# lefarov/Ape-X-DQN

Measured on AMD Instinct MI355X. Metric: learner grad-steps/sec at batch 512, 84x84x4 dueling DQN, higher is better.
Workload: dtype fp32; 1 GPU; model=dueling NatureCNN (reference DuellingDQN, conv1=64), 4x84x84, A=4, global_batch=512, seq_len=1, parallelism=dp1, batch_scope=global, per_rank_rows=512, replay_per_gpu=100000, learner=fused/hip, hip_graphs=True

## Files before the change

apex_dqn_amd/csrc/sumtree.hip:

```cpp
#include "apex_common.h"
#include <stdlib.h>
#include "head_common.h"
#include "igemm_wgrad.h"
#include "rmsprop_common.h"
#include "pack_rows.h"

#define APEX_DBG_SITES 8
#ifdef APEX_DEBUG_BOUNDS
__device__ int apex_dbg_count[APEX_DBG_SITES];
__device__ long long apex_dbg_first[APEX_DBG_SITES];
__device__ __forceinline__ bool apex_dbg_ok(int64_t i, int64_t n, int site) {
  if (i >= 0 && i < n) return true;
  if (atomicAdd(&apex_dbg_count[site], 1) == 0) apex_dbg_first[site] = (long long)i;
  return false;
}
#define APEX_DBG_OK(i, n, site) apex_dbg_ok((int64_t)(i), (int64_t)(n), site)
#define APEX_DBG_CLAMP(i, n, site) (APEX_DBG_OK(i, n, site) ? (i) : ((i) < 0 ? 0 : (n) - 1))
#else
#define APEX_DBG_OK(i, n, site) true
#define APEX_DBG_CLAMP(i, n, site) (i)
#endif

struct TreeDesc {
  float* leaf;
// ... 525 lines not shown
  if (n <= 0 && ctr_to_bump == nullptr) return 0;
  if (dedupe && n > 1024) return (int)hipErrorInvalidValue;
  const int threads = n <= 1024 ? ((n + 63) / 64) * 64 : 1024;
  const int nb = n > 0 ? blocks_for(n, threads) : 1;
  tree_update_kernel<<<nb, threads > 0 ? threads : 64, 0, st>>>(t, idx, values, n, mode, alpha, eps, gen_expect,
                                                               gen, dedupe, ctr_to_bump, tree_kfirst(t));
  APEX_CHECK_LAUNCH();
}

APEX_EXPORT int apex_tree_zero_range(TreeDesc t, int64_t start, int64_t count, hipStream_t st) {
  if (count <= 0) return 0;
  tree_zero_range_kernel<<<blocks_for(count, 256), 256, 0, st>>>(t, start, count, tree_kfirst(t));
  APEX_CHECK_LAUNCH();
}

APEX_EXPORT int apex_replay_insert(TreeDesc t, RecordDesc r, int64_t start, int K, const int32_t* s_obs,
                                   const int32_t* s_nxt, const int32_t* s_act, const float* s_rew,
                                   const float* s_gam, const float* s_prio, float alpha, float eps,
                                   hipStream_t st) {
  if (K <= 0) return 0;
  replay_insert_kernel<<<blocks_for(K, 256), 256, 0, st>>>(t, r, start, K, s_obs, s_nxt, s_act, s_rew,
                                                           s_gam, s_prio, alpha, eps, tree_kfirst(t));
  APEX_CHECK_LAUNCH();
}

APEX_EXPORT int apex_tree_sample(TreeDesc t, RecordDesc r, int B, uint64_t seed, const uint64_t* ctr,
                                 float beta, int64_t* out_idx, float* out_w,
                                 int32_t* out_gen, int32_t* out_obs, int32_t* out_nxt, int32_t* out_act,
                                 float* out_rew, float* out_gam, int32_t* out_nxt2, const double* shard_stats,
                                 int shard_rank, int shard_world, uint64_t shard_seed, float* out_wscale,
                                 int64_t mcap, hipStream_t st) {
  if (B <= 0) return 0;
  if (mcap <= 0) mcap = (int64_t)shard_world * B;
  if (shard_stats != nullptr && (B < 3 || shard_world < 1 || shard_rank < 0 || shard_rank >= shard_world))
    return (int)hipErrorInvalidValue;
  const int waves_per_block = 4;
  tree_sample_kernel<<<blocks_for(B, waves_per_block), 64 * waves_per_block, 0, st>>>(
      SampleArgs{t, r, B, seed, ctr, beta, out_idx, out_w, out_gen, out_obs, out_nxt, out_act,
                 out_rew, out_gam, out_nxt2, shard_stats, shard_rank, shard_world, shard_seed, out_wscale,
                 mcap});
  APEX_CHECK_LAUNCH();
}

APEX_EXPORT int apex_tree_rebuild(TreeDesc t, hipStream_t st) {
  fill_u32_kernel<<<1, 64, 0, st>>>(t.min_bits, 0x7f800000u, 1);
  for (int k = 1; k <= t.L; ++k) {
    int64_t nd = t.n[k];
    const int wpb = 4;
    if (k == 1) {
      const int nb = blocks_for(nd, wpb);
      tree_reduce_leaf_kernel<<<nb < 512 ? nb : 512, 64 * wpb, 0, st>>>(t.leaf, t.n[0], t.nodes + t.off[1], nd,
                                                                       t.min_bits);
      continue;
    }
    tree_reduce_level_kernel<<<blocks_for(nd, wpb), 64 * wpb, 0, st>>>(
        nullptr, t.nodes + t.off[k - 1], t.n[k - 1], t.nodes + t.off[k], nd, t.min_bits);
  }
  APEX_CHECK_LAUNCH();
}

APEX_EXPORT int apex_gather_frames(const uint8_t* ring, const int32_t* slots, int n_slots, int64_t nframes,
                                   int64_t frame_bytes, uint8_t* out, hipStream_t st) {
  if (n_slots <= 0) return 0;
  if (frame_bytes % 16) return (int)hipErrorInvalidValue;
  gather_frames_kernel<<<n_slots, 256, 0, st>>>(ring, slots, nframes, frame_bytes, out);
  APEX_CHECK_LAUNCH();
}

__global__ void fill16_kernel(uint4* p, int64_t n, int nt) {
  typedef uint32_t u32x4v __attribute__((ext_vector_type(4)));
  const uint4 v = make_uint4(1u, 1u, 1u, 1u);
  const u32x4v vv = {1u, 1u, 1u, 1u};
  for (int64_t i = (int64_t)blockIdx.x * blockDim.x + threadIdx.x; i < n; i += (int64_t)gridDim.x * blockDim.x) {
    if (nt) __builtin_nontemporal_store(vv, reinterpret_cast<u32x4v*>(p + i));
    else p[i] = v;
  }
}

APEX_EXPORT int apex_fill16(void* p, int64_t n, int nt, hipStream_t st) {
  fill16_kernel<<<2048, 256, 0, st>>>(reinterpret_cast<uint4*>(p), n, nt);
  APEX_CHECK_LAUNCH();
}

APEX_EXPORT int apex_abi_version() { return 8; }

APEX_EXPORT int apex_debug_bounds_enabled() {
#ifdef APEX_DEBUG_BOUNDS
  return 1;
#else
  return 0;
#endif
}

APEX_EXPORT int apex_debug_errors(int* counts, long long* first, int reset) {
#ifdef APEX_DEBUG_BOUNDS
  hipError_t e = hipDeviceSynchronize();
  if (e != hipSuccess) return (int)e;
  e = hipMemcpyFromSymbol(counts, HIP_SYMBOL(apex_dbg_count), sizeof(int) * APEX_DBG_SITES);
  if (e != hipSuccess) return (int)e;
  e = hipMemcpyFromSymbol(first, HIP_SYMBOL(apex_dbg_first), sizeof(long long) * APEX_DBG_SITES);
  if (e != hipSuccess) return (int)e;
  if (reset) {
    int zc[APEX_DBG_SITES] = {0};
    long long zf[APEX_DBG_SITES] = {0};
    hipMemcpyToSymbol(HIP_SYMBOL(apex_dbg_count), zc, sizeof(zc));
    e = hipMemcpyToSymbol(HIP_SYMBOL(apex_dbg_first), zf, sizeof(zf));
  }
  return (int)e;
#else
  for (int i = 0; i < APEX_DBG_SITES; ++i) {
    counts[i] = 0;
    first[i] = 0;
  }
  return 0;
#endif
}

APEX_EXPORT int apex_rmsprop_sample(float* p, const float* g, float* v, float* m, bf16_t* pb, int64_t n,
                                    const double* partials, int npart, float lr, float alpha, float eps_opt,
                                    float clip, int centered, float* norm_out, TreeDesc t, RecordDesc r, int B,
                                    uint64_t seed, const uint64_t* ctr, float beta,
                                    int64_t* out_idx, float* out_w, int32_t* out_gen, int32_t* out_obs,
                                    int32_t* out_nxt, int32_t* out_act, float* out_rew, float* out_gam,
                                    int32_t* out_nxt2, const double* shard_stats, int shard_rank, int shard_world,
                                    uint64_t shard_seed, float* out_wscale, int64_t mcap, bf16_t* pb_lo,
                                    const double* wnorm, int wn, int wstride, CfFragOut fo, const RmsSegs* seg,
                                    const float* gpre, int64_t npre, hipStream_t st) {
  if (mcap <= 0) mcap = (int64_t)shard_world * B;
  if (shard_stats != nullptr && (B < 3 || shard_world < 1 || shard_rank < 0 || shard_rank >= shard_world))
    return (int)hipErrorInvalidValue;
  if (((uintptr_t)p | (uintptr_t)g | (uintptr_t)v | (uintptr_t)m) & 15) return (int)hipErrorInvalidValue;
  if ((((uintptr_t)pb | (uintptr_t)pb_lo) & 7) || B < 0) return (int)hipErrorInvalidValue;
  constexpr int nt = 512, maxb = 256;
  int nb = (int)((n / 4 + nt - 1) / nt);
  nb = nb < 1 ? 1 : (nb > maxb ? maxb : nb);
  RmsSegs sg{};
  if (seg != nullptr) {
    sg = *seg;
    if (sg.nseg < 1 || sg.nseg > 3) return (int)hipErrorInvalidValue;
    int64_t tot = 0;
    for (int k = 0; k < sg.nseg; ++k) {
      if ((sg.off[k] & 3) || sg.len[k] <= 0 || sg.off[k] < 0 || sg.off[k] + sg.len[k] > n)
        return (int)hipErrorInvalidValue;
      tot += sg.len[k];
    }
    const int64_t fend = fo.c3f != nullptr && fo.w3_off + 36864 > fo.w2_off + 65536 ? fo.w3_off + 36864
                                                                                     : fo.w2_off + 65536;
    const int64_t need0 = fo.w1frag != nullptr ? fend / 4 / nt + 1 : 1;
    int b0 = 0;
    for (int k = 0; k < sg.nseg; ++k) {
      const int64_t full = (sg.len[k] / 4 + nt - 1) / nt;
      int64_t nbk = (int64_t)maxb * sg.len[k] / tot;
      if (k == 0 && nbk < need0) nbk = need0;
      if (nbk > full) nbk = full;
      if (nbk < 1) nbk = 1;
      sg.blk0[k] = b0;
      b0 += (int)nbk;
    }
    sg.blk0[sg.nseg] = b0;
    nb = sg.blk0[1];
  }
  const int nsb = B > 0 ? blocks_for(B, nt / 64) : 0;
  const int64_t n0 = seg != nullptr ? sg.len[0] : n;
  if (fo.w1frag != nullptr && (seg != nullptr && sg.off[0] != 0)) return (int)hipErrorInvalidValue;
  if (fo.w1frag != nullptr && (fo.c2f == nullptr || (fo.C != 1 && fo.C != 2 && fo.C != 4) ||
                               (fo.w1_off & 3) || (fo.w2_off & 7) || fo.w1_off + 4096LL * fo.C > n0 ||
                               fo.w2_off + 65536 > n0 ||
// ... 65 lines not shown
```

apex_dqn_amd/ops/_lib.py:

```python
from __future__ import annotations

import ctypes
import os
from typing import Optional

import torch

from . import build as _build

c_p = ctypes.c_void_p
c_i = ctypes.c_int
c_i64 = ctypes.c_int64
c_u64 = ctypes.c_uint64
c_f = ctypes.c_float


class TreeDesc(ctypes.Structure):
    _fields_ = [("leaf", c_p), ("nodes", c_p), ("off", c_i64 * 8), ("n", c_i64 * 8), ("L", c_i),
                ("min_bits", c_p)]


class RecordDesc(ctypes.Structure):
    _fields_ = [("obs", c_p), ("nxt", c_p), ("act", c_p), ("rew", c_p), ("gam", c_p), ("gen", c_p),
                ("C", c_i), ("cap", c_i64), ("nframes", c_i64)]
# ... 57 lines not shown
                ("nsplit", c_i), ("nb", c_i), ("s2dC", c_i), ("Kc", c_i), ("scale", c_f), ("blk0", c_i),
                ("cpb", c_i), ("jnorm", c_p)]


class FinalizeDesc(ctypes.Structure):
    _fields_ = [("job", RedJob * 4), ("njobs", c_i), ("nrm_n", c_i), ("nrm_ptr", c_p), ("norm_part", c_p),
                ("norm_slot0", c_i), ("nblocks", c_i)]


class Conv1WgDesc(ctypes.Structure):
    _fields_ = [("ring", c_p), ("slots", c_p), ("dy", c_p), ("slab", c_p), ("bias_slab", c_p), ("zero16", c_p),
                ("N", c_i), ("C", c_i), ("dy_lo", c_p), ("wq", c_p)]


class Conv1S2DDesc(ctypes.Structure):
    _fields_ = [("ring", c_p), ("slots", c_p), ("w", c_p), ("w2", c_p), ("bias", c_p), ("bias2", c_p),
                ("y", c_p), ("zero16", c_p), ("scratch", c_p), ("N", c_i), ("C", c_i), ("m_switch", c_i),
                ("in_scale", c_f), ("probe", c_p), ("w32", c_p), ("w2_32", c_p), ("y_lo", c_p),
                ("c2f_src", c_p * 4), ("c2f_out", c_p), ("c2f_bf16", c_i)]


_SIGS = {
    "apex_abi_version": ([], c_i),
    "apex_build_id": ([], ctypes.c_char_p),
    "apex_fill16": ([c_p, c_i64, c_i, c_p], c_i),
    "apex_tree_update": ([TreeDesc, c_p, c_p, c_i, c_i, c_f, c_f, c_p, c_p, c_i, c_p, c_p], c_i),
    "apex_tree_zero_range": ([TreeDesc, c_i64, c_i64, c_p], c_i),
    "apex_replay_insert": ([TreeDesc, RecordDesc, c_i64, c_i, c_p, c_p, c_p, c_p, c_p, c_p, c_f, c_f, c_p],
                           c_i),
    "apex_tree_sample": ([TreeDesc, RecordDesc, c_i, c_u64, c_p, c_f, c_p, c_p, c_p, c_p, c_p, c_p, c_p,
                          c_p, c_p, c_p, c_i, c_i, c_u64, c_p, c_i64, c_p], c_i),
    "apex_tree_rebuild": ([TreeDesc, c_p], c_i),
    "apex_gather_frames": ([c_p, c_p, c_i, c_i64, c_i64, c_p, c_p], c_i),
    "apex_debug_bounds_enabled": ([], c_i),
    "apex_debug_errors": ([c_p, c_p, c_i], c_i),
    "apex_grad_sqnorm_partials": ([c_p, c_i64, c_p, c_p], c_i),
    "apex_rmsprop_step": ([c_p, c_p, c_p, c_p, c_p, c_i64, c_p, c_f, c_f, c_f, c_f, c_i, c_p, c_p, c_p, c_i, c_i,
                           c_p], c_i),
    "apex_cast_bf16": ([c_p, c_p, c_i64, c_p, c_p], c_i),
    "apex_spin_hold": ([c_i, c_i, c_i, c_p, c_p], c_i),
    "apex_rmsprop_step_np": ([c_p, c_p, c_p, c_p, c_p, c_i64, c_p, c_i, c_f, c_f, c_f, c_f, c_i, c_p, c_p, c_p,
                              c_i, c_i, c_p], c_i),
    "apex_grad_finalize": ([FinalizeDesc, c_p], c_i),
    "apex_norm_total": ([c_p, c_i, c_p, c_p], c_i),
    "apex_ddqn_head": ([c_p, c_p, HeadParams, HeadParams, c_p, c_p, c_p, c_p, c_i, c_i, c_i, c_f, c_f, c_p,
                        c_p, c_p, c_p, c_p, c_p, c_i, c_i, HeadLo, HeadPart, C2dPack, IsNorm, c_p], c_i),
    "apex_rmsprop_sample": ([c_p, c_p, c_p, c_p, c_p, c_i64, c_p, c_i, c_f, c_f, c_f, c_f, c_i, c_p,
                             TreeDesc, RecordDesc, c_i, c_u64, c_p, c_f, c_p, c_p, c_p, c_p, c_p, c_p, c_p, c_p,
                             c_p, c_p, c_i, c_i, c_u64, c_p, c_i64, c_p, c_p, c_i, c_i, CfFragOut, c_p, c_p, c_i64,
                             c_p], c_i),
    "apex_head_wgrad_prio": ([c_p, c_p, c_i, c_i, c_p, c_p, c_p, c_p, c_i, TreeDesc, c_p, c_p, c_p, c_p, c_f, c_f,
                              c_p, c_p, c_p, c_p, c_p, c_p, c_i, c_i, c_p, c_i64, c_p], c_i),
    "apex_fc_wgrad_head_prio": ([WgradDesc, c_p, c_p, c_i, c_i, c_p, c_p, c_p, c_p, c_i, TreeDesc, c_p, c_p, c_p,
                                 c_p, c_f, c_f, c_p, c_p, c_p, c_p], c_i),
    "apex_head_wgrad": ([c_p, c_p, c_i, c_i, c_p, c_p, c_p, c_p, c_i, c_p, c_p], c_i),
    "apex_actor_head": ([c_p, HeadParams, c_i, c_i, c_p, c_u64, c_p, c_p, c_p, c_i, c_p, c_p], c_i),
    "apex_conv1_s2d_fwd": ([Conv1S2DDesc, c_i, c_p], c_i),
    "apex_conv1_wgrad_img": ([Conv1WgDesc, c_i, c_p], c_i),
    "apex_slab_reduce": ([c_p, c_i, c_i64, c_f, c_p, c_p, c_i, c_p, c_i, c_i, c_p], c_i),
    "apex_s2d_pack_w1": ([c_p, c_p, c_i, c_p], c_i),
    "apex_s2d_unpack_w1_grad": ([c_p, c_p, c_i, c_p], c_i),
    "apex_s2d_frames": ([c_p, c_p, c_i64, c_i64, c_i64, c_p], c_i),
    "apex_atari_frames": ([c_p, c_p, c_i64, c_i64, c_i64, c_p], c_i),
    "apex_pack_rows": ([c_p, c_p, c_p, c_i, c_i, c_p, c_i64, c_p], c_i),
    "apex_sqnorm_ranges": ([c_p, c_i64, c_p, c_i64, c_p, c_i, c_p], c_i),
    "apex_copy_segments": ([c_i, c_p, c_p, c_p, c_p], c_i),
}

_LIB: Optional[ctypes.CDLL] = None
_LOAD_ERROR: Optional[str] = None


def _declare(lib: ctypes.CDLL) -> None:
    for name, (args, res) in _SIGS.items():
        fn = getattr(lib, name, None)
        if fn is None:
            continue
        fn.argtypes = args
        fn.restype = res
    from . import conv_sigs
    conv_sigs.declare(lib)


ABI_VERSION = 8


def load(build_if_missing: bool = True) -> Optional[ctypes.CDLL]:
    global _LIB, _LOAD_ERROR
    if _LIB is not None:
        return _LIB
    debug = debug_bounds_requested()
    try:
        path = _build.ensure_current("kernels_debug" if debug else "kernels", allow_build=build_if_missing)
        lib = ctypes.CDLL(path, mode=ctypes.RTLD_LOCAL)
        _declare(lib)
        if lib.apex_abi_version() != ABI_VERSION:
            raise RuntimeError(f"{path}: ABI {lib.apex_abi_version()} != {ABI_VERSION}")
        _LIB = lib
    except Exception as e:
        _LOAD_ERROR = repr(e)
        _LIB = None
    return _LIB


def debug_bounds_requested() -> bool:
    return os.environ.get("APEX_DEBUG_BOUNDS", "0") not in ("", "0")


DEBUG_SITES = ("tree_update.leaf", "replay_insert.slot", "tree_sample.slot", "gather_frames.frame",
               "replay_insert.frame_value", "tree_zero_range.slot", "unused6", "unused7")


def debug_errors(reset: bool = True) -> dict:
    lib = require_kernels()
    counts = (ctypes.c_int * 8)()
    first = (ctypes.c_longlong * 8)()
    check(lib.apex_debug_errors(ctypes.addressof(counts), ctypes.addressof(first), int(reset)), "debug_errors")
    return {DEBUG_SITES[i]: (int(counts[i]), int(first[i])) for i in range(8) if counts[i]}


def available() -> bool:
    return load() is not None


def require_kernels() -> ctypes.CDLL:
    lib = load()
    if lib is None:
        raise RuntimeError(f"apex HIP kernel library unavailable: {_LOAD_ERROR}. "
                           f"Run `python -m apex_dqn_amd.ops.build`.")
    return lib


def stream_ptr(device: Optional[torch.device] = None) -> int:
    return torch.cuda.current_stream(device).cuda_stream


def ptr(t: Optional[torch.Tensor]) -> Optional[int]:
    return None if t is None else t.data_ptr()


def head_lo(Hon_lo=None, Htg_lo=None, dH_lo=None) -> HeadLo:
    lo = HeadLo()
    lo.Hon, lo.Htg, lo.dH = ptr(Hon_lo), ptr(Htg_lo), ptr(dH_lo)
    return lo


def check(rc: int, what: str) -> None:
    if rc != 0:
        raise RuntimeError(f"{what} failed with hipError {rc}")
```

apex_dqn_amd/ops/conv.py:

```python
from __future__ import annotations

from typing import Dict, Optional, Tuple


import torch

from . import _lib
from .switches import SW


class Workspace:
    def __init__(self):
        self.bufs: Dict[Tuple, torch.Tensor] = {}

    def get(self, key, numel: int, device, dtype=torch.float32) -> torch.Tensor:
        k = (key, numel, str(device), dtype)
        t = self.bufs.get(k)
        if t is None:
            t = torch.empty(numel, dtype=dtype, device=device)
            self.bufs[k] = t
        return t

    work_queue = False

# ... 324 lines not shown
def conv3_dgrad_img(lib, dy: torch.Tensor, w3: torch.Tensor, mask: torch.Tensor, out: torch.Tensor,
                    grid: int = 0) -> None:
    from .conv_sigs import Conv3DgradImgDesc
    N = dy.shape[0]
    assert tuple(dy.shape) == (N, 7, 7, 64) and tuple(out.shape) == (N, 9, 9, 64)
    assert tuple(mask.shape) == (N, 9, 9, 64) and tuple(w3.shape) == (64, 3, 3, 64)
    assert dy.is_contiguous() and out.is_contiguous() and mask.is_contiguous() and w3.is_contiguous()
    d = Conv3DgradImgDesc()
    d.dy, d.w, d.mask, d.dx, d.N = dy.data_ptr(), w3.data_ptr(), mask.data_ptr(), out.data_ptr(), N
    _lib.check(lib.apex_conv3_dgrad_img(d, int(grid), _lib.stream_ptr()), "conv3_dgrad_img")


def conv3_dgrad(lib, dy: torch.Tensor, w3: torch.Tensor, mask: torch.Tensor, out: torch.Tensor, dy_lo=None,
                w_lo=None, out_lo=None) -> None:
    N = dy.shape[0]
    assert w3.shape == (64, 3, 3, 64)
    if SW.conv3_dgrad_img and dy_lo is None and hasattr(lib, "apex_conv3_dgrad_img"):
        conv3_dgrad_img(lib, dy, w3, mask, out)
        return
    d = _conv_desc(x=dy.data_ptr(), w=w3.data_ptr(), y=out.data_ptr(), mask=mask.data_ptr(), N=N, H=7, W=7,
                   Cin=64, OH=9, OW=9, Cout=64, KH=3, KW=3, stride=1, pad=2, mode=1, K=576,
                   bt=1, ldb=576, koff=_KOFF3, **_lo(dy_lo, w_lo, None, out_lo))
    _launch_fwd(lib, d)


def conv2_dgrad_img(lib, dy: torch.Tensor, w2: torch.Tensor, mask: torch.Tensor, out: torch.Tensor,
                    grid: int = 0, dy_lo=None, w_lo=None, out_lo=None, ws: Optional["Workspace"] = None,
                    packed: bool = False) -> None:
    from .conv_sigs import Conv2DgradImgDesc
    N = dy.shape[0]
    assert tuple(dy.shape) == (N, 9, 9, 64) and tuple(out.shape) == (N, 20, 20, 64)
    assert tuple(mask.shape) == (N, 20, 20, 64) and tuple(w2.shape) == (64, 4, 4, 64)
    assert dy.is_contiguous() and out.is_contiguous() and mask.is_contiguous() and w2.is_contiguous()
    d = Conv2DgradImgDesc()
    d.dy, d.w, d.mask, d.dx, d.N = dy.data_ptr(), w2.data_ptr(), mask.data_ptr(), out.data_ptr(), N
    if dy_lo is not None:
        for t in (dy_lo, w_lo, out_lo):
            assert t is not None and t.is_contiguous() and t.dtype == torch.bfloat16
        d.dy_lo, d.w_lo, d.dx_lo = dy_lo.data_ptr(), w_lo.data_ptr(), out_lo.data_ptr()
    ws = ws if ws is not None else _DEFAULT_WS
    d.wfrag = c2d_wfrag_buffer(ws, dy.device).data_ptr()
    d.wfrag_ready = int(packed)
    d.wq = ws.wq(("c2d_wq", N, int(grid)), dy.device)
    d.cls_split = int(dy_lo is not None and N <= SW.conv2_dgrad_cls_max)
    _lib.check(lib.apex_conv2_dgrad_img(d, int(grid), _lib.stream_ptr()), "conv2_dgrad_img")


def conv2_dgrad(lib, dy: torch.Tensor, w2: torch.Tensor, mask: torch.Tensor, out: torch.Tensor, dy_lo=None,
                w_lo=None, out_lo=None, ws: Optional["Workspace"] = None, packed: bool = False) -> None:
    N = dy.shape[0]
    assert w2.shape == (64, 4, 4, 64)
    if SW.conv2_dgrad_img and hasattr(lib, "apex_conv2_dgrad_img"):
        conv2_dgrad_img(lib, dy, w2, mask, out, dy_lo=dy_lo, w_lo=w_lo, out_lo=out_lo, ws=ws, packed=packed)
        return
    d = _conv_desc(x=dy.data_ptr(), w=w2.data_ptr(), y=out.data_ptr(), mask=mask.data_ptr(), N=N, H=9, W=9,
                   Cin=64, OH=10, OW=10, Cout=64, KH=2, KW=2, stride=1, pad=1, mode=1, K=256, ncls=4,
                   ostride=2, OHfull=20, OWfull=20, bt=1, ldb=1024, koff=_KOFF2, **_lo(dy_lo, w_lo, None, out_lo))
    _launch_fwd(lib, d)


def _wg_desc(**kw) -> "_lib.WgradDesc":
    d = _lib.WgradDesc()
    d.dy, d.x, d.frame_slots = kw["dy"], kw["x"], kw.get("frame_slots")
    d.slab, d.bias_slab = kw["slab"], kw.get("bias_slab")
    d.N, d.H, d.W, d.Cin = kw.get("N", 1), kw.get("H", 1), kw.get("W", 1), kw.get("Cin", 64)
    d.OH, d.OW, d.KH, d.KW = kw.get("OH", 1), kw.get("OW", 1), kw.get("KH", 1), kw.get("KW", 1)
    d.stride, d.pad_h, d.pad_w, d.mode = kw.get("stride", 1), 0, 0, kw["mode"]
    d.Co, d.Kc, d.ldd, d.ldx = kw["Co"], kw["Kc"], kw["ldd"], kw.get("ldx", 0)
    d.rows_per_split, d.Mred = kw["rows_per_split"], kw["Mred"]
    d.norm_part, d.norm_slot0 = kw.get("norm_part"), kw.get("norm_slot0", 0)
    d.dy_lo, d.x_lo = kw.get("dy_lo"), kw.get("x_lo")
    return d


_WG_ROWS = 64
_WG_TBL = 1024


def _splits(Mred: int, target_rows: int, max_rows: int) -> Tuple[int, int]:
    rows = max(_WG_ROWS, min(max_rows, (target_rows // _WG_ROWS) * _WG_ROWS))
    return (Mred + rows - 1) // rows, rows


def conv_wgrad(lib, ws: Workspace, dy: torch.Tensor, x: torch.Tensor, KH: int, stride: int,
               dw_out: torch.Tensor, db_out: torch.Tensor, target_rows: int = 0, jobs: Optional[list] = None,
               dy_lo=None, x_lo=None) -> None:
    N, OH, OW, Co = dy.shape
    if target_rows <= 0:
        small = N < 256
        target_rows = {3: SW.wg_rows3, 4: SW.wg_rows2}.get(KH) or \
            ((192 if small else 384) if KH == 3 else (352 if small else 704))
    _, H, W, Cin = x.shape
    Kc = KH * KH * Cin
    Mred = N * OH * OW
    nsplit, rows = _splits(Mred, target_rows, _WG_TBL)
    slab = ws.get(("wg", Co, Kc), nsplit * Co * Kc, dy.device)
    bslab = ws.get(("wgb", Co, Kc), nsplit * Co, dy.device)
    d = _wg_desc(dy=dy.data_ptr(), x=x.data_ptr(), slab=slab.data_ptr(), bias_slab=bslab.data_ptr(), N=N,
                 H=H, W=W, Cin=Cin, OH=OH, OW=OW, KH=KH, KW=KH, stride=stride, mode=1, Co=Co, Kc=Kc, ldd=Co,
                 rows_per_split=rows, Mred=Mred, dy_lo=_lib.ptr(dy_lo), x_lo=_lib.ptr(x_lo))
    if jobs is not None:
        _lib.check(lib.apex_conv_wgrad(d, None, None, nsplit, 1.0, _lib.stream_ptr()), "conv_wgrad")
        jobs.append(dict(slab=slab, bslab=bslab, out=dw_out, bout=db_out, n=Co * Kc, nsplit=nsplit, nb=Co,
                         s2dC=0, Kc=Kc, scale=1.0))
        return
    _lib.check(lib.apex_conv_wgrad(d, dw_out.data_ptr(), db_out.data_ptr(), nsplit, 1.0, _lib.stream_ptr()),
               "conv_wgrad")


def conv1_wgrad_ring(lib, ws: Workspace, dy: torch.Tensor, ring: torch.Tensor, slots: torch.Tensor,
                     scale: float, dw_out: torch.Tensor, db_out: torch.Tensor, grid: int = 0,
                     jobs: Optional[list] = None, dy_lo: Optional[torch.Tensor] = None) -> None:
    N, OH, OW, Co = dy.shape
    C = slots.shape[1]
    assert (OH, OW, Co) == (20, 20, 64) and slots.dtype == torch.int32 and dy.is_contiguous()
    G = grid if grid > 0 else min(N, 256)
    K = 64 * C
    slab = ws.get(("wg1img", C, G), G * 64 * K, dy.device)
    bslab = ws.get(("wg1imgb", G), G * 64, dy.device)
    zero = ws.get(("zero16",), 64, ring.device, torch.uint8)
    if not getattr(ws, "_zeroed", False):
        zero.zero_()
        ws._zeroed = True
    d = _lib.Conv1WgDesc()
    d.ring, d.slots, d.dy = ring.data_ptr(), slots.data_ptr(), dy.data_ptr()
    d.slab, d.bias_slab, d.zero16 = slab.data_ptr(), bslab.data_ptr(), zero.data_ptr()
    d.N, d.C = N, C
    d.dy_lo = _lib.ptr(dy_lo)
    d.wq = ws.wq(("c1w_wq", N, int(G)), dy.device)
    st = _lib.stream_ptr()
    _lib.check(lib.apex_conv1_wgrad_img(d, G, st), "conv1_wgrad_img")
    if jobs is not None:
        jobs.append(dict(slab=slab, bslab=bslab, out=dw_out, bout=db_out, n=64 * K, nsplit=G, nb=64, s2dC=C, Kc=K,
                         scale=float(scale)))
        return
    _lib.check(lib.apex_slab_reduce(slab.data_ptr(), G, 64 * K, float(scale), dw_out.data_ptr(), bslab.data_ptr(),
                                    64, db_out.data_ptr(), C, K, st), "slab_reduce")


def conv2_dgrad_conv1_wgrad_fused(lib, ws: Workspace, dy: torch.Tensor, dy_lo: torch.Tensor, w2: torch.Tensor,
                                  w_lo: torch.Tensor, mask: torch.Tensor, ring: torch.Tensor, slots: torch.Tensor,
                                  scale: float, dw_out: torch.Tensor, db_out: torch.Tensor, grid: int = 0,
                                  jobs: Optional[list] = None, packed: bool = False,
                                  dx: Optional[torch.Tensor] = None, dx_lo: Optional[torch.Tensor] = None,
                                  wq: int = 0) -> None:
    from .conv_sigs import Conv21BwdDesc
    N = dy.shape[0]
    C = slots.shape[1]
    assert tuple(dy.shape) == (N, 9, 9, 64) and tuple(mask.shape) == (N, 20, 20, 64)
    assert tuple(w2.shape) == (64, 4, 4, 64) and slots.dtype == torch.int32 and slots.shape[0] == N
    assert dy.is_contiguous() and mask.is_contiguous() and w2.is_contiguous() and slots.is_contiguous()
    for t in (dy_lo, w_lo):
        assert t is not None and t.is_contiguous() and t.dtype == torch.bfloat16
    for t in (dx, dx_lo):
        assert t is None or (tuple(t.shape) == (N, 20, 20, 64) and t.is_contiguous() and t.dtype == torch.bfloat16)
    G = grid if grid > 0 else min(N, 256)
    K = 64 * C
    slab = ws.get(("wg1img", C, G), G * 64 * K, dy.device)
    bslab = ws.get(("wg1imgb", G), G * 64, dy.device)
    zero = ws.get(("zero16",), 64, ring.device, torch.uint8)
    if not getattr(ws, "_zeroed", False):
        zero.zero_()
        ws._zeroed = True
    d = Conv21BwdDesc()
    d.dy, d.dy_lo, d.w, d.w_lo, d.mask = dy.data_ptr(), dy_lo.data_ptr(), w2.data_ptr(), w_lo.data_ptr(), mask.data_ptr()
    d.wfrag = c2d_wfrag_buffer(ws, dy.device).data_ptr()
    d.wfrag_ready = int(packed)
    d.ring, d.slots, d.zero16 = ring.data_ptr(), slots.data_ptr(), zero.data_ptr()
    d.slab, d.bias_slab = slab.data_ptr(), bslab.data_ptr()
    d.dx, d.dx_lo = _lib.ptr(dx), _lib.ptr(dx_lo)
    d.wq = wq or None
    d.N, d.C = N, C
    st = _lib.stream_ptr()
    _lib.check(lib.apex_conv21_bwd_fused(d, G, st), "conv21_bwd_fused")
    if jobs is not None:
        jobs.append(dict(slab=slab, bslab=bslab, out=dw_out, bout=db_out, n=64 * K, nsplit=G, nb=64, s2dC=C, Kc=K,
                         scale=float(scale)))
        return
    _lib.check(lib.apex_slab_reduce(slab.data_ptr(), G, 64 * K, float(scale), dw_out.data_ptr(), bslab.data_ptr(),
                                    64, db_out.data_ptr(), C, K, st), "slab_reduce")


def conv1_wgrad_ring_tiled(lib, ws: Workspace, dy: torch.Tensor, ring: torch.Tensor, slots: torch.Tensor,
                           scale: float, dw_out: torch.Tensor, db_out: torch.Tensor, target_rows: int = 0,
                           jobs: Optional[list] = None, dy_lo: Optional[torch.Tensor] = None) -> None:
    if target_rows <= 0:
        target_rows = 800 if dy_lo is not None else 1024
    N, OH, OW, Co = dy.shape
    C = slots.shape[1]
    Kc = C * 64
# ... 131 lines not shown
```

apex_dqn_amd/ops/conv_sigs.py:

```python
from __future__ import annotations

import ctypes

c_p = ctypes.c_void_p
c_i = ctypes.c_int
c_i64 = ctypes.c_int64
c_f = ctypes.c_float


class Conv2ImgDesc(ctypes.Structure):
    _fields_ = [("x", c_p), ("w", c_p), ("w2", c_p), ("bias", c_p), ("bias2", c_p), ("y", c_p),
                ("N", c_i), ("img_switch", c_i), ("x_lo", c_p), ("w_lo", c_p), ("w2_lo", c_p), ("y_lo", c_p),
                ("wfrag", c_p), ("wfrag_ready", c_i)]


class Conv12Desc(ctypes.Structure):
    _fields_ = [("ring", c_p), ("slots", c_p), ("w1", c_p), ("w1b", c_p), ("b1", c_p), ("b1b", c_p),
                ("w2", c_p), ("w2_lo", c_p), ("w2b", c_p), ("w2b_lo", c_p), ("wfrag", c_p), ("pack_sets", c_i),
                ("b2", c_p), ("b2b", c_p), ("y1", c_p), ("y1_lo", c_p), ("y2", c_p), ("y2_lo", c_p),
                ("w1frag", c_p), ("scratch", c_p), ("N", c_i), ("C", c_i), ("img_switch", c_i), ("copy_n", c_i),
                ("in_scale", ctypes.c_float), ("probe", c_p), ("wq", c_p), ("bf16", c_i), ("probe_split", c_i),
                ("w3", c_p), ("w3_lo", c_p), ("w3b", c_p), ("w3b_lo", c_p), ("b3", c_p), ("b3b", c_p),
                ("y3", c_p), ("y3_lo", c_p), ("w3frag", c_p)]


class Conv2DgradImgDesc(ctypes.Structure):
    _fields_ = [("dy", c_p), ("w", c_p), ("mask", c_p), ("dx", c_p), ("N", c_i), ("dy_lo", c_p), ("w_lo", c_p),
                ("dx_lo", c_p), ("wfrag", c_p), ("wfrag_ready", c_i), ("wq", c_p), ("cls_split", c_i)]


class Conv21BwdDesc(ctypes.Structure):
    _fields_ = [("dy", c_p), ("dy_lo", c_p), ("w", c_p), ("w_lo", c_p), ("mask", c_p), ("wfrag", c_p),
                ("wfrag_ready", c_i), ("ring", c_p), ("slots", c_p), ("zero16", c_p), ("slab", c_p),
                ("bias_slab", c_p), ("dx", c_p), ("dx_lo", c_p), ("wq", c_p), ("N", c_i), ("C", c_i)]


class C2dPackJob(ctypes.Structure):
    _fields_ = [("w", c_p), ("w_lo", c_p), ("out", c_p)]


class Conv3DgradImgDesc(ctypes.Structure):
    _fields_ = [("dy", c_p), ("w", c_p), ("mask", c_p), ("dx", c_p), ("N", c_i)]


def declare(lib: ctypes.CDLL) -> None:
    from ._lib import ConvDesc, WgradDesc
    sigs = {
        "apex_conv2_img_fwd": ([Conv2ImgDesc, c_i, c_p], c_i),
        "apex_conv12_fused_fwd": ([Conv12Desc, c_i, c_p], c_i),
        "apex_conv12_pack": ([Conv12Desc, c_p], c_i),
        "apex_conv2_dgrad_img": ([Conv2DgradImgDesc, c_i, c_p], c_i),
        "apex_conv3_dgrad_img": ([Conv3DgradImgDesc, c_i, c_p], c_i),
        "apex_conv21_bwd_fused": ([Conv21BwdDesc, c_i, c_p], c_i),
        "apex_conv_fwd": ([ConvDesc, c_p], c_i),
        "apex_fc_gemm128": ([ConvDesc, c_p, c_i64, c_i, c_i, c_i, C2dPackJob, c_p], c_i),
        "apex_conv_wgrad": ([WgradDesc, c_p, c_p, c_i, c_f, c_p], c_i),
        "apex_pack_dgrad_weights": ([c_p, c_p, c_p, c_p, c_p, c_p, c_p], c_i),
    }
    for name, (args, res) in sigs.items():
        fn = getattr(lib, name, None)
        if fn is None:
            continue
        fn.argtypes = args
        fn.restype = res
```

apex_dqn_amd/ops/switches.py:

```python
from __future__ import annotations

import dataclasses
import os
from dataclasses import dataclass
from typing import Any, Dict


@dataclass
class Switches:
    conv2_img: bool = True
    c2f_pack: bool = True
    conv12_fused: bool = True
    conv123_max_images: int = 1 << 20
    conv12_bf16: bool = True
    conv3_dgrad_img: bool = True
    conv2_dgrad_img: bool = True
    conv2_dgrad_cls_max: int = 256
    conv21_bwd_fused: bool = True
    opt_frags: bool = True
    fc_epi_in_head: bool = True
    bwd_branches: bool = True
    actor_fc_ksplit: int = 4
    fc_wgrad_main: str = "auto"
    fc_ksplit_max: int = 0
    work_queue: str = "auto"
    wg_rows3: int = 0
    wg_rows2: int = 0
    impala_wg_target: int = 512
    impala_slab_cap: int = 8 << 20
    resblock_r16: int = 14
    impala_pool_wgrad: bool = True
    isplit_bands: str = ""
    dp_fc_shard_branch: bool = False
    dp_branch_one_wait: bool = True
    dp_fc_split_rows: int = -1
    dp_norm_split: bool = True

    @classmethod
    def from_env(cls, spec: str = None) -> "Switches":
        sw = cls()
        spec = os.environ.get("APEX_SWITCHES", "") if spec is None else spec
        for item in spec.split(","):
            item = item.strip()
            if not item:
                continue
            if "=" not in item:
                raise ValueError(f"APEX_SWITCHES item must be name=value, got {item!r}")
            k, v = item.split("=", 1)
            f = {f.name: f for f in dataclasses.fields(cls)}.get(k)
            if f is None:
                raise ValueError(f"unknown kernel switch {k!r}")
            setattr(sw, k, _parse(f.type, v))
        return sw

    def non_default(self) -> Dict[str, Any]:
        d = Switches()
        return {f.name: getattr(self, f.name) for f in dataclasses.fields(self)
                if getattr(self, f.name) != getattr(d, f.name)}


def _parse(typ, v: str):
    t = typ if isinstance(typ, str) else typ.__name__
    if t == "bool":
        return v.lower() not in ("0", "false", "off", "no")
    if t == "int":
        return int(v)
    return v


SW = Switches.from_env()
```

Before: 2837 grad-steps/s (batch 512).

## Add specialised conv2 weight-gradient kernel with row-ring LDS reuse

Adds a dedicated conv2 (4x4 stride 2, 20x20x64 to 9x9x64) weight-gradient kernel. It streams input rows into an LDS ring buffer with async DMA and reuses them across output rows for each kh, with one workgroup per kh per split. It uses a precomputed row table and split bf16 hi/lo MFMA accumulation. It replaces the generic implicit-GEMM wgrad when batch is at least 512 and both lo buffers are present. The aim is to avoid redundant global reads of overlapping im2col patches, at the cost of a four-times larger grid and extra complexity.

```diff
diff --git a/apex_dqn_amd/csrc/conv2_wgrad_rows.hip b/apex_dqn_amd/csrc/conv2_wgrad_rows.hip
--- /dev/null
+++ b/apex_dqn_amd/csrc/conv2_wgrad_rows.hip
@@ -0,0 +1,218 @@
+#include "igemm_wgrad.h"
+
+#define C2R_D 24
+#define C2R_SLOT 5120
+#define C2R_CELLS (C2R_D * 40)
+#define C2R_LO 2560
+#define C2R_ZERO (C2R_D * C2R_SLOT)
+#define C2R_DY (C2R_ZERO + 21 * 128)
+#define C2R_DYSTAGE (2 * WG_IMG)
+#define C2R_TBL (C2R_DY + 2 * C2R_DYSTAGE)
+#define C2R_MAXROWS 1024
+#define C2R_SMEM (C2R_TBL + 2 * C2R_MAXROWS * 2)
+
+__device__ __forceinline__ int c2r_f(int v) { return ((v >> 1) & 1) | (((v >> 3) & 1) << 1); }
+
+__global__ void __launch_bounds__(512) conv2_wgrad_rows_kernel(WgradDesc d) {
+  static_assert(C2R_SMEM <= 163840, "LDS");
+  static_assert((C2R_D & 1) == 0 && C2R_D >= 16, "ring: whole 1-KB pieces, two steps' rows");
+  __shared__ __attribute__((aligned(256))) uint8_t smem[C2R_SMEM];
+  const int tid = threadIdx.x, lane = tid & 63;
+  const int wv = __builtin_amdgcn_readfirstlane(tid >> 6);
+  const int half = wv >> 2, kw = wv & 3;
+  const int wg = xcd_swizzle((int)blockIdx.x, (int)gridDim.x);
+  const int kh = wg & 3, split = wg >> 2;
+  const int r_begin = split * d.rows_per_split;
+  const int r_end = min(d.Mred, r_begin + d.rows_per_split);
+  const int nst = (r_end - r_begin + WG_ROWS - 1) / WG_ROWS;
+  const int trows = nst * WG_ROWS;
+  const int J0 = r_begin / 9, Jlast = (r_end - 1) / 9;
+
+  uint16_t* tbl = reinterpret_cast<uint16_t*>(smem + C2R_TBL);
+  for (int r = tid; r < trows; r += 512) {
+    const int m = r_begin + r;
+    uint32_t e0 = C2R_CELLS, e1 = C2R_CELLS;
+    if (m < r_end) {
+      const int J = m / 9, ow = m - 9 * J;
+      const int base = ((J - J0) % C2R_D) * 40;
+      e0 = (uint32_t)(base + (ow ^ (J & 1))) | ((uint32_t)c2r_f(m) << 12);
+      e1 = (uint32_t)(base + ((ow + 1) ^ (J & 1))) | ((uint32_t)c2r_f(m + 1) << 12);
+    }
+    tbl[r] = (uint16_t)e0;
+    tbl[C2R_MAXROWS + r] = (uint16_t)e1;
+  }
+  if (tid < 8) {
+    *reinterpret_cast<uint4*>(smem + C2R_ZERO + tid * 16) = make_uint4(0, 0, 0, 0);
+    *reinterpret_cast<uint4*>(smem + C2R_ZERO + C2R_LO + tid * 16) = make_uint4(0, 0, 0, 0);
+  }
+
+  const uint32_t lds0 = (uint32_t)(uintptr_t)(__attribute__((address_space(3))) uint8_t*)smem;
+  const uint8_t* xh = static_cast<const uint8_t*>(d.x);
+  const uint8_t* xl = static_cast<const uint8_t*>(d.x_lo);
+  auto issue_piece = [&](int Q) {
+    const int jr = Q / 5, k = Q - 5 * jr, J = J0 + jr;
+    const int sc = 8 * k + (lane >> 3);
+    const int plane = sc >= 20 ? 1 : 0, w20 = sc - 20 * plane;
+    const int e = w20 >= 10 ? 1 : 0, u = (w20 - 10 * e) ^ (J & 1);
+    const int c = (lane & 7) ^ (c2r_f(9 * J + u) << 1);
+    const int img = J / 9, oh = J - 9 * img;
+    const size_t off = ((size_t)((img * 20 + 2 * oh + kh) * 20 + 2 * u + e) << 7) + (size_t)(c << 4);
+    const uint32_t l = lds0 + (uint32_t)((jr % C2R_D) * C2R_SLOT + k * 1024);
+    dma16((plane ? xl : xh) + off, __builtin_amdgcn_readfirstlane(l));
+  };
+  auto issue_pieces = [&](int Qa, int Qb) -> int {
+    int n = 0;
+    for (int Q = Qa + ((wv - Qa) & 7); Q < Qb; Q += 8, ++n) issue_piece(Q);
+    return n;
+  };
+  const int srow = tid >> 3;
+  const int sc8 = (tid & 7) ^ ((((srow >> 1) & 1) | (((srow >> 3) & 1) << 1)) << 1);
+  const __amdgpu_buffer_rsrc_t dy_rs =
+      __builtin_amdgcn_make_buffer_rsrc(const_cast<bf16_t*>(d.dy), (short)0, r_end * 128, 0x00020000);
+  const __amdgpu_buffer_rsrc_t dyl_rs =
+      __builtin_amdgcn_make_buffer_rsrc(const_cast<bf16_t*>(d.dy_lo), (short)0, r_end * 128, 0x00020000);
+  const uint32_t dy_off = (uint32_t)((r_begin + srow) * 128 + sc8 * 16);
+  auto issue_dy = [&](int st) {
+    const uint32_t o = dy_off + (uint32_t)st * (WG_ROWS * 128);
+    const uint32_t l = __builtin_amdgcn_readfirstlane(lds0 + C2R_DY + (uint32_t)(st & 1) * C2R_DYSTAGE + (uint32_t)wv * 1024u);
+    bdma16(dy_rs, o, l);
+    bdma16(dyl_rs, o, l + WG_IMG);
+  };
+  auto jhi = [&](int st) { return (min(r_end, r_begin + WG_ROWS * (st + 1)) - 1) / 9; };
+  auto jlo = [&](int st) { return (r_begin + WG_ROWS * st) / 9; };
+
+  const int g = lane >> 4, q = (lane >> 2) & 3, pcol = lane & 3, pl = lane & 15;
+  const int rA = 32 * half + 8 * g + q;
+  const uint16_t* trow = tbl + (kw >> 1) * C2R_MAXROWS + rA;
+  const int eoff = (kw & 1) * 1280 + 8 * pcol;
+  const bool do_bias = d.bias_slab != nullptr && kh == 0 && kw == 0;
+  f32x4 acc[4][4], accb[4];
+#pragma unroll
+  for (int a = 0; a < 4; ++a) {
+    accb[a] = (f32x4){0.f, 0.f, 0.f, 0.f};
+#pragma unroll
+    for (int b = 0; b < 4; ++b) acc[a][b] = (f32x4){0.f, 0.f, 0.f, 0.f};
+  }
+  const bf16x8 ones = __builtin_bit_cast(bf16x8, make_uint4(0x3f803f80u, 0x3f803f80u, 0x3f803f80u, 0x3f803f80u));
+
+  auto xfrag = [&](int a0, int f0, int a1, int f1, int t) -> bf16x8 {
+    const lds_s16x4* pa = (const lds_s16x4*)(smem + a0 + ((t ^ f0) << 5));
+    const lds_s16x4* pb = (const lds_s16x4*)(smem + a1 + ((t ^ f1) << 5));
+    const s16x4 lo = __builtin_amdgcn_ds_read_tr16_b64_v4i16(const_cast<lds_s16x4*>(pa));
+    const s16x4 hi = __builtin_amdgcn_ds_read_tr16_b64_v4i16(const_cast<lds_s16x4*>(pb));
+    typedef short s16x8 __attribute__((ext_vector_type(8)));
+    const s16x8 v = (s16x8){lo[0], lo[1], lo[2], lo[3], hi[0], hi[1], hi[2], hi[3]};
+    return __builtin_bit_cast(bf16x8, v);
+  };
+
+  uint32_t e0 = 0, e1 = 0;
+  auto compute = [&](int st) {
+    if (st == 0) e0 = trow[0], e1 = trow[4];
+    const int c0 = e0 & 0xfff, c1 = e1 & 0xfff, f0 = e0 >> 12, f1 = e1 >> 12;
+    const int a0 = (c0 << 7) + (c0 < C2R_CELLS ? eoff : 8 * pcol);
+    const int a1 = (c1 << 7) + (c1 < C2R_CELLS ? eoff : 8 * pcol);
+    const uint8_t* D = smem + C2R_DY + (st & 1) * C2R_DYSTAGE;
+    const uint8_t* DL = D + WG_IMG;
+    if (st + 1 < nst) e0 = trow[(st + 1) * WG_ROWS], e1 = trow[(st + 1) * WG_ROWS + 4];
+    bf16x8 a[4], b[4], al[4], bl[4];
+#pragma unroll
+    for (int t = 0; t < 4; ++t) {
+      a[t] = tr_frag8(D, half, 16 * t, lane);
+      al[t] = tr_frag8(DL, half, 16 * t, lane);
+    }
+#pragma unroll
+    for (int t = 0; t < 4; ++t) {
+      b[t] = xfrag(a0, f0, a1, f1, t);
+      bl[t] = xfrag(a0 + C2R_LO, f0, a1 + C2R_LO, f1, t);
+    }
+#pragma unroll
+    for (int i = 0; i < 4; ++i)
+#pragma unroll
+      for (int j = 0; j < 4; ++j) {
+        acc[i][j] = __builtin_amdgcn_mfma_f32_16x16x32_bf16(b[j], al[i], acc[i][j], 0, 0, 0);
+        acc[i][j] = __builtin_amdgcn_mfma_f32_16x16x32_bf16(bl[j], a[i], acc[i][j], 0, 0, 0);
+        acc[i][j] = __builtin_amdgcn_mfma_f32_16x16x32_bf16(b[j], a[i], acc[i][j], 0, 0, 0);
+      }
+    if (do_bias) {
+#pragma unroll
+      for (int i = 0; i < 4; ++i) {
+        accb[i] = __builtin_amdgcn_mfma_f32_16x16x32_bf16(ones, al[i], accb[i], 0, 0, 0);
+        accb[i] = __builtin_amdgcn_mfma_f32_16x16x32_bf16(ones, a[i], accb[i], 0, 0, 0);
+      }
+    }
+  };
+
+  int Qn = 0;
+  int ahead;
+  {
+    const int q1 = 5 * (jhi(0) - J0 + 1), q3 = 5 * (min(Jlast, J0 + C2R_D - 1) - J0 + 1);
+    issue_pieces(0, q1);
+    issue_dy(0);
+    ahead = issue_pieces(q1, q3);
+    Qn = q3;
+  }
+  for (int st = 0; st < nst; ++st) {
+    vmcnt_le(ahead);
+    __syncthreads();
+    ahead = 0;
+    if (st + 1 < nst) {
+      const int q1 = max(Qn, 5 * (jhi(st + 1) - J0 + 1));
+      const int q3 = max(q1, 5 * (min(Jlast, jlo(st) + C2R_D - 1) - J0 + 1));
+      issue_pieces(Qn, q1);
+      issue_dy(st + 1);
+      ahead = issue_pieces(q1, q3);
+      Qn = q3;
+    }
+    compute(st);
+  }
+
+  vmcnt_le(0);
+  __syncthreads();
+  f32x4* red = reinterpret_cast<f32x4*>(smem) + kw * (20 * 64) + lane;
+  if (half) {
+#pragma unroll
+    for (int k = 0; k < 16; ++k) red[k * 64] = acc[k >> 2][k & 3];
+#pragma unroll
+    for (int i = 0; i < 4; ++i) red[(16 + i) * 64] = accb[i];
+  }
+  __syncthreads();
+  if (half) return;
+#pragma unroll
+  for (int k = 0; k < 16; ++k) acc[k >> 2][k & 3] += red[k * 64];
+#pragma unroll
+  for (int i = 0; i < 4; ++i) accb[i] += red[(16 + i) * 64];
+
+  float* slab = d.slab + (int64_t)split * 64 * 1024;
+#pragma unroll
+  for (int i = 0; i < 4; ++i)
+#pragma unroll
+    for (int j = 0; j < 4; ++j)
+      *reinterpret_cast<f32x4*>(slab + (16 * i + pl) * 1024 + (kh * 4 + kw) * 64 + 16 * j + 4 * g) = acc[i][j];
+  if (do_bias && g == 0) {
+#pragma unroll
+    for (int i = 0; i < 4; ++i) d.bias_slab[(int64_t)split * 64 + 16 * i + pl] = accb[i][0];
+  }
+}
+
+static bool conv2_wgrad_rows_covers(const WgradDesc& d) {
+  return d.mode == 1 && d.H == 20 && d.W == 20 && d.Cin == 64 && d.OH == 9 && d.OW == 9 && d.KH == 4 &&
+         d.KW == 4 && d.stride == 2 && d.pad_h == 0 && d.pad_w == 0 && d.Co == 64 && d.Kc == 1024 &&
+         d.ldd == 64 && d.dy_lo != nullptr && d.x_lo != nullptr && d.norm_part == nullptr &&
+         d.rows_per_split > 0 && (d.rows_per_split & 63) == 0 && d.rows_per_split <= C2R_MAXROWS &&
+         d.N > 0 && d.Mred == d.N * 81 && (int64_t)d.Mred * 128 < 0x7ffffff0LL;
+}
+
+APEX_EXPORT int apex_slab_reduce(const float* slab, int nsplit, int64_t n, float scale, float* out, const float* bslab,
+                                 int nb, float* bout, int s2dC, int Kc, hipStream_t st);
+
+APEX_EXPORT int apex_conv2_wgrad_rows(WgradDesc d, float* out, float* bout, int nsplit, float scale, hipStream_t st) {
+  if (!conv2_wgrad_rows_covers(d)) return (int)hipErrorInvalidValue;
+  if (nsplit != (d.Mred + d.rows_per_split - 1) / d.rows_per_split) return (int)hipErrorInvalidValue;
+  conv2_wgrad_rows_kernel<<<4 * nsplit, 512, 0, st>>>(d);
+  hipError_t e = hipGetLastError();
+  if (e != hipSuccess) return (int)e;
+  if (out != nullptr)
+    return apex_slab_reduce(d.slab, nsplit, (int64_t)64 * 1024, scale, out, d.bias_slab, d.bias_slab ? 64 : 0, bout, 0,
+                            1024, st);
+  return 0;
+}
diff --git a/apex_dqn_amd/csrc/sumtree.hip b/apex_dqn_amd/csrc/sumtree.hip
--- a/apex_dqn_amd/csrc/sumtree.hip
+++ b/apex_dqn_amd/csrc/sumtree.hip
@@ -631,7 +631,7 @@
   APEX_CHECK_LAUNCH();
 }
 
-APEX_EXPORT int apex_abi_version() { return 8; }
+APEX_EXPORT int apex_abi_version() { return 9; }
 
 APEX_EXPORT int apex_debug_bounds_enabled() {
 #ifdef APEX_DEBUG_BOUNDS
diff --git a/apex_dqn_amd/ops/_lib.py b/apex_dqn_amd/ops/_lib.py
--- a/apex_dqn_amd/ops/_lib.py
+++ b/apex_dqn_amd/ops/_lib.py
@@ -163,7 +163,7 @@
     conv_sigs.declare(lib)
 
 
-ABI_VERSION = 8
+ABI_VERSION = 9
 
 
 def load(build_if_missing: bool = True) -> Optional[ctypes.CDLL]:
diff --git a/apex_dqn_amd/ops/conv.py b/apex_dqn_amd/ops/conv.py
--- a/apex_dqn_amd/ops/conv.py
+++ b/apex_dqn_amd/ops/conv.py
@@ -430,9 +430,26 @@
     return (Mred + rows - 1) // rows, rows
 
 
+def conv2_wgrad_rows_covers(x_shape, dy_shape, KH: int, stride: int, split: bool, rows: int) -> bool:
+    return (bool(split) and KH == 4 and stride == 2 and len(x_shape) == 4 and len(dy_shape) == 4
+            and tuple(x_shape[1:]) == (20, 20, 64) and tuple(dy_shape[1:]) == (9, 9, 64)
+            and x_shape[0] == dy_shape[0] and x_shape[0] > 0
+            and rows > 0 and rows % _WG_ROWS == 0 and rows <= _WG_TBL)
+
+
+def conv2_wgrad_rows_pick(x_shape, dy_shape, KH: int, stride: int, split: bool, rows: int,
+                          force: Optional[bool] = None) -> bool:
+    covers = conv2_wgrad_rows_covers(x_shape, dy_shape, KH, stride, split, rows)
+    if force is not None:
+        if force and not covers:
+            raise ValueError("conv2_wgrad_rows does not cover this problem")
+        return bool(force)
+    return covers and bool(SW.conv2_wgrad_rows) and x_shape[0] >= SW.conv2_wgrad_rows_min
+
+
 def conv_wgrad(lib, ws: Workspace, dy: torch.Tensor, x: torch.Tensor, KH: int, stride: int,
                dw_out: torch.Tensor, db_out: torch.Tensor, target_rows: int = 0, jobs: Optional[list] = None,
-               dy_lo=None, x_lo=None) -> None:
+               dy_lo=None, x_lo=None, rows_kernel: Optional[bool] = None) -> None:
     N, OH, OW, Co = dy.shape
     if target_rows <= 0:
         small = N < 256
@@ -447,13 +464,16 @@
     d = _wg_desc(dy=dy.data_ptr(), x=x.data_ptr(), slab=slab.data_ptr(), bias_slab=bslab.data_ptr(), N=N,
                  H=H, W=W, Cin=Cin, OH=OH, OW=OW, KH=KH, KW=KH, stride=stride, mode=1, Co=Co, Kc=Kc, ldd=Co,
                  rows_per_split=rows, Mred=Mred, dy_lo=_lib.ptr(dy_lo), x_lo=_lib.ptr(x_lo))
+    launch, what = lib.apex_conv_wgrad, "conv_wgrad"
+    if conv2_wgrad_rows_pick(x.shape, dy.shape, KH, stride, dy_lo is not None and x_lo is not None, rows,
+                             rows_kernel):
+        launch, what = lib.apex_conv2_wgrad_rows, "conv2_wgrad_rows"
     if jobs is not None:
-        _lib.check(lib.apex_conv_wgrad(d, None, None, nsplit, 1.0, _lib.stream_ptr()), "conv_wgrad")
+        _lib.check(launch(d, None, None, nsplit, 1.0, _lib.stream_ptr()), what)
         jobs.append(dict(slab=slab, bslab=bslab, out=dw_out, bout=db_out, n=Co * Kc, nsplit=nsplit, nb=Co,
                          s2dC=0, Kc=Kc, scale=1.0))
         return
-    _lib.check(lib.apex_conv_wgrad(d, dw_out.data_ptr(), db_out.data_ptr(), nsplit, 1.0, _lib.stream_ptr()),
-               "conv_wgrad")
+    _lib.check(launch(d, dw_out.data_ptr(), db_out.data_ptr(), nsplit, 1.0, _lib.stream_ptr()), what)
 
 
 def conv1_wgrad_ring(lib, ws: Workspace, dy: torch.Tensor, ring: torch.Tensor, slots: torch.Tensor,
diff --git a/apex_dqn_amd/ops/conv_sigs.py b/apex_dqn_amd/ops/conv_sigs.py
--- a/apex_dqn_amd/ops/conv_sigs.py
+++ b/apex_dqn_amd/ops/conv_sigs.py
@@ -55,6 +55,7 @@
         "apex_conv_fwd": ([ConvDesc, c_p], c_i),
         "apex_fc_gemm128": ([ConvDesc, c_p, c_i64, c_i, c_i, c_i, C2dPackJob, c_p], c_i),
         "apex_conv_wgrad": ([WgradDesc, c_p, c_p, c_i, c_f, c_p], c_i),
+        "apex_conv2_wgrad_rows": ([WgradDesc, c_p, c_p, c_i, c_f, c_p], c_i),
         "apex_pack_dgrad_weights": ([c_p, c_p, c_p, c_p, c_p, c_p, c_p], c_i),
     }
     for name, (args, res) in sigs.items():
diff --git a/apex_dqn_amd/ops/switches.py b/apex_dqn_amd/ops/switches.py
--- a/apex_dqn_amd/ops/switches.py
+++ b/apex_dqn_amd/ops/switches.py
@@ -26,6 +26,8 @@
     work_queue: str = "auto"
     wg_rows3: int = 0
     wg_rows2: int = 0
+    conv2_wgrad_rows: bool = True
+    conv2_wgrad_rows_min: int = 512
     impala_wg_target: int = 512
     impala_slab_cap: int = 8 << 20
     resblock_r16: int = 14
```

Measured after the change: 2869 grad-steps/s (batch 512) (median of 6 runs). +1.1%, better.
